# mbzuai-metaverse/XMem2

Hardware: AMD Instinct MI355X
Metric: frames/sec at 480p, 1 obj, 32 memory frames; mask IoU vs reference (higher is better)
Workload: dtype f32

## Files before the change

xmem2_amd/csrc/gemm_stream.hip:

```cpp
#include "gemm_stream.hpp"
#include <stdlib.h>

#ifdef XMEM_TOOLS
#define DBG(bit) (p.dbg & (bit))
#else
#define DBG(bit) 0
#endif

namespace {

__device__ __forceinline__ void glds16(const void* sbase, unsigned voff, unsigned lds_addr) {
    asm volatile("s_mov_b32 m0, %0\n\ts_nop 0\n\tglobal_load_lds_dwordx4 %1, %2" : : "s"(lds_addr), "v"(voff), "s"(sbase) : "memory");
}

template <int N>
__device__ __forceinline__ void wait_loads_only() {
    asm volatile("s_waitcnt vmcnt(%0)" : : "n"(N) : "memory");
}

template <int N>
__device__ __forceinline__ void wait_loads_then_barrier() {
    asm volatile("s_waitcnt vmcnt(%0)\n\ts_barrier" : : "n"(N) : "memory");
}

template <int TM, int TN, int NS, int MODE>
__global__ __launch_bounds__(256) void gemm_stream_kernel(GemmStreamArgs p) {
    constexpr int BM = 64 * TM, BN = 64 * TN;
    constexpr int STAGE = (BM + BN) * 128;
    constexpr int LA = BM / 32, LB = BN / 32;
    constexpr int L = LA + LB;
    extern __shared__ __attribute__((aligned(16))) unsigned char smem[];

    const int tid = threadIdx.x, lane = tid & 63;
    const int wave = __builtin_amdgcn_readfirstlane(tid >> 6);
    const int wm = wave >> 1, wn = wave & 1;
    const int l31 = lane & 31, lh = lane >> 5;

    int bid = blockIdx.x;
    {
        const int nwg = gridDim.x, q = nwg >> 3, r = nwg & 7, xcd = bid & 7;
        bid = (xcd < r ? xcd * (q + 1) : r * (q + 1) + (xcd - r) * q) + (bid >> 3);
    }
    const int ustep = DBG(32) ? 1 : (int)gridDim.x;
    const int u0 = DBG(32) ? bid * p.units_per_wg : bid;
    const int u1 = DBG(32) ? min(p.units, u0 + p.units_per_wg) : p.units;
    if (u0 >= u1) return;
    const int nunits = (u1 - u0 + ustep - 1) / ustep;
    const int S = nunits * p.nk;
    const unsigned lds_base = (unsigned)(size_t)smem;

    const int lrow = lane >> 3, lslot = lane & 7;
    unsigned a_voff[LA], b_voff[LB];
    int ld_u = u0, ld_kt = 0;
    const char* ld_abase = nullptr;
    const char* ld_bbase = nullptr;
    auto ld_unit_setup = [&]() {
        const int lu = DBG(1) ? 0 : ld_u;
        const int tn = lu % p.tiles_n, t2 = lu / p.tiles_n;
        const int tm = t2 % p.tiles_m, g = t2 / p.tiles_m;
        const int m0 = tm * BM, n0 = tn * BN;
#pragma unroll
        for (int i = 0; i < LA; ++i) {
            const int r = 8 * (4 * i + wave) + lrow;
            const int m = min(m0 + r, p.M - 1);
            unsigned row = (unsigned)m;
            if (MODE == 1 && p.stride != 1) {
                const int b = m / p.HoWo, rem = m - b * p.HoWo;
                const int oh = rem / p.Wo, ow = rem - oh * p.Wo;
                row = (unsigned)((b * p.H + oh * p.stride) * p.W + ow * p.stride);
            }
            a_voff[i] = (row * (unsigned)p.lda + (unsigned)((lslot ^ ((r >> 1) & 7)) * 4)) * 4u;
        }
#pragma unroll
        for (int i = 0; i < LB; ++i) {
            const int r = 8 * (4 * i + wave) + lrow;
            const int n = min(n0 + r, p.N - 1);
            b_voff[i] = ((unsigned)n * (unsigned)p.ldb + (unsigned)((lslot ^ ((r >> 1) & 7)) * 4)) * 4u;
        }
        ld_abase = reinterpret_cast<const char*>(p.A + (size_t)g * p.a_gstride);
        ld_bbase = reinterpret_cast<const char*>(p.B + (size_t)g * p.b_gstride);
    };
    auto issue = [&](int stage) {
        const char* ab = ld_abase + (size_t)ld_kt * 128;
        const char* bb = ld_bbase + (size_t)ld_kt * 128;
        const unsigned dst = lds_base + (unsigned)stage * STAGE + (unsigned)wave * 1024u;
#pragma unroll
        for (int i = 0; i < LA; ++i) glds16(ab, a_voff[i], dst + i * 4096);
#pragma unroll
        for (int i = 0; i < LB; ++i) glds16(bb, b_voff[i], dst + BM * 128 + i * 4096);
        if (++ld_kt == p.nk) {
            ld_kt = 0;
            ld_u += ustep;
            if (ld_u < u1) ld_unit_setup();
        }
    };

    const int swz = (l31 >> 1) & 7;
    unsigned rd_a[4], rd_b[4];
#pragma unroll
    for (int kk = 0; kk < 4; ++kk) {
        const unsigned ch = (unsigned)(((2 * kk + lh) ^ swz) * 16);
        rd_a[kk] = (unsigned)((wm * 32 * TM + l31) * 128) + ch;
        rd_b[kk] = (unsigned)(BM * 128 + (wn * 32 * TN + l31) * 128) + ch;
    }

    ld_unit_setup();
#pragma unroll
    for (int j = 0; j < NS - 1; ++j)
        if (j < S) issue(j);

    constexpr int ST = (MODE == 0) ? 16 * TM * TN : 0;
    constexpr int WAIT_STEADY = L * (NS - 2);
    constexpr int WAIT_CREDIT = (WAIT_STEADY + ST > 63) ? 63 : WAIT_STEADY + ST;
    int s = 0, stage = 0, credit = 0;
    for (int cu = u0; cu < u1; cu += ustep) {
        f32x16 acc[TM][TN];
#pragma unroll
        for (int i = 0; i < TM; ++i)
#pragma unroll
            for (int j = 0; j < TN; ++j)
#pragma unroll
                for (int r = 0; r < 16; ++r) acc[i][j][r] = 0.f;

        for (int kt = 0; kt < p.nk; ++kt, ++s) {
            const int behind = S - 1 - s;
            if (DBG(4)) wait_loads_only<WAIT_STEADY>();
            else if (behind >= NS - 2) {
                if (ST > 0 && credit > 0) wait_loads_then_barrier<WAIT_CREDIT>();
                else wait_loads_then_barrier<WAIT_STEADY>();
            } else if (NS > 3 && behind == 1) wait_loads_then_barrier<L>();
            else wait_loads_then_barrier<0>();
            if (credit > 0) --credit;
            if (s + NS - 1 < S && !DBG(8)) {
                int st = stage + NS - 1; if (st >= NS) st -= NS;
                issue(st);
            }

            const unsigned char* sb = smem + (DBG(16) ? 0 : stage * STAGE);
            f32x4 af[2][TM], bf[2][TN];
            if (DBG(16)) {
                const f32x4 c = {1.f, 2.f, 3.f, 4.f};
#pragma unroll
                for (int i = 0; i < TM; ++i) { af[0][i] = c; af[1][i] = c; }
#pragma unroll
                for (int j = 0; j < TN; ++j) { bf[0][j] = c; bf[1][j] = c; }
#pragma unroll
                for (int kk = 0; kk < 4; ++kk)
#pragma unroll
                    for (int t = 0; t < 4; ++t)
#pragma unroll
                        for (int i = 0; i < TM; ++i)
#pragma unroll
                            for (int j = 0; j < TN; ++j)
                                acc[i][j] = __builtin_amdgcn_mfma_f32_32x32x2f32(af[0][i][t], bf[0][j][t], acc[i][j], 0, 0, 0);
                if (++stage == NS) stage = 0;
                continue;
            }
#pragma unroll
            for (int i = 0; i < TM; ++i) af[0][i] = *reinterpret_cast<const f32x4*>(sb + rd_a[0] + i * 4096);
#pragma unroll
            for (int j = 0; j < TN; ++j) bf[0][j] = *reinterpret_cast<const f32x4*>(sb + rd_b[0] + j * 4096);
#pragma unroll
            for (int kk = 0; kk < 4; ++kk) {
                const int cur = kk & 1, nxt = cur ^ 1;
                if (kk + 1 < 4) {
#pragma unroll
                    for (int i = 0; i < TM; ++i) af[nxt][i] = *reinterpret_cast<const f32x4*>(sb + rd_a[kk + 1] + i * 4096);
#pragma unroll
                    for (int j = 0; j < TN; ++j) bf[nxt][j] = *reinterpret_cast<const f32x4*>(sb + rd_b[kk + 1] + j * 4096);
                }
                __builtin_amdgcn_sched_barrier(0);
                if (MODE == 1) {
#pragma unroll
                    for (int i = 0; i < TM; ++i) {
                        af[cur][i].x = fmaxf(af[cur][i].x, p.relu_in ? 0.f : af[cur][i].x); af[cur][i].y = fmaxf(af[cur][i].y, p.relu_in ? 0.f : af[cur][i].y);
                        af[cur][i].z = fmaxf(af[cur][i].z, p.relu_in ? 0.f : af[cur][i].z); af[cur][i].w = fmaxf(af[cur][i].w, p.relu_in ? 0.f : af[cur][i].w);
                    }
                }
#pragma unroll
                for (int t = 0; t < 4; ++t)
#pragma unroll
                    for (int i = 0; i < TM; ++i)
#pragma unroll
                        for (int j = 0; j < TN; ++j)
                            acc[i][j] = __builtin_amdgcn_mfma_f32_32x32x2f32(af[cur][i][t], bf[cur][j][t], acc[i][j], 0, 0, 0);
            }
            if (++stage == NS) stage = 0;
        }

        const int tn = cu % p.tiles_n, t2 = cu / p.tiles_n;
        const int tm = t2 % p.tiles_m, g = t2 / p.tiles_m;
        const int m0 = tm * BM, n0 = tn * BN;
        float* const cg = p.C + (size_t)g * p.c_gstride;
        bool all_full = true;
        if (DBG(2)) { credit = 0; continue; }
#pragma unroll
        for (int j = 0; j < TN; ++j) {
            const int nb = n0 + wn * 32 * TN + j * 32;
            const int n = nb + l31;
            float sc = 1.f, sh = 0.f;
            if (MODE == 1 && n < p.N) { sc = p.scale[n]; sh = p.shift[n]; }
#pragma unroll
            for (int i = 0; i < TM; ++i) {
                const int mw = m0 + wm * 32 * TM + i * 32;
                const int mb = mw + 4 * lh;
                float* const orow = cg + (size_t)mb * p.ldc + n;
                const bool full = (mw + 32 <= p.M) && (nb + 32 <= p.N);
                all_full = all_full && full;
                if (MODE == 0) {
                    if (full) {
#pragma unroll
                        for (int r = 0; r < 16; ++r) orow[(size_t)((r & 3) + 8 * (r >> 2)) * p.ldc] = acc[i][j][r];
                    } else if (n < p.N) {
#pragma unroll
                        for (int r = 0; r < 16; ++r) {
                            const int o = (r & 3) + 8 * (r >> 2);
                            if (mb + o < p.M) orow[(size_t)o * p.ldc] = acc[i][j][r];
                        }
                    }
                } else if (n < p.N) {
                    float rv[16];
                    if (p.res) {
#pragma unroll
                        for (int r = 0; r < 16; ++r) {
                            const int o = (r & 3) + 8 * (r >> 2);
                            const int t = p.res_mod ? (mb + o) % p.res_mod : min(mb + o, p.M - 1);
                            rv[r] = p.res[(size_t)t * p.ldres + n];
                        }
                    }
                    float vout[16];
#pragma unroll
                    for (int r = 0; r < 16; ++r) {
                        float v = acc[i][j][r] * sc + sh;
                        if (p.res) v += rv[r];
                        vout[r] = p.relu_out ? fmaxf(v, 0.f) : v;
                    }
#pragma unroll
                    for (int r = 0; r < 16; ++r) {
                        const int o = (r & 3) + 8 * (r >> 2);
                        if (mb + o < p.M) orow[(size_t)o * p.ldc] = vout[r];
                    }
                }
            }
        }
        credit = (ST > 0 && all_full) ? NS - 1 : 0;
    }
}

template <int TM, int TN, int NS>
int launch_variant(const GemmStreamArgs& a, int nwg, hipStream_t s) {
    const size_t lds = (size_t)NS * (64 * TM + 64 * TN) * 128;
    auto kern = a.mode == 1 ? gemm_stream_kernel<TM, TN, NS, 1> : gemm_stream_kernel<TM, TN, NS, 0>;
    if (xmem_ensure_dynamic_lds(reinterpret_cast<const void*>(kern), lds) != XMEM_OK) return XMEM_ERR_LAUNCH;
    hipLaunchKernelGGL(kern, dim3(nwg), dim3(256), lds, s, a);
    return xmem_check_launch();
}

}

size_t gemm_stream_lds_bytes(int variant, int ring) {
    const int bm = variant == 0 ? 64 : 128, bn = variant == 2 ? 128 : 64;
    return (size_t)ring * (bm + bn) * 128;
}

int gemm_stream_launch(GemmStreamArgs& a, int variant, int ring, hipStream_t s) {
    if (a.K % 32 != 0 || a.K <= 0 || a.M <= 0 || a.N <= 0 || a.G <= 0) return XMEM_ERR_UNSUPPORTED;
    if (variant < 0 || variant > 2 || (ring != 3 && ring != 4)) return XMEM_ERR_BAD_ARG;
    const int bm = variant == 0 ? 64 : 128, bn = variant == 2 ? 128 : 64;
    a.dbg = 0;
#ifdef XMEM_TOOLS
    { static const int dbg = getenv("XMEM_STREAM_DBG") ? atoi(getenv("XMEM_STREAM_DBG")) : 0; a.dbg = dbg; }
#endif
    a.nk = a.K / 32;
    a.tiles_m = cdiv(a.M, bm); a.tiles_n = cdiv(a.N, bn);
    const long units = (long)a.G * a.tiles_m * a.tiles_n;
    if (units > 0x7fffffff) return XMEM_ERR_UNSUPPORTED;
    a.units = (int)units;
    const size_t lds = gemm_stream_lds_bytes(variant, ring);
    int per_cu = (int)((160 * 1024) / lds); if (per_cu > 8) per_cu = 8; if (per_cu < 1) per_cu = 1;
    const int slots = 256 * per_cu;
    a.units_per_wg = cdiv(a.units, slots);
    const int nwg = cdiv(a.units, a.units_per_wg);
    if (variant == 0) return ring == 3 ? launch_variant<1, 1, 3>(a, nwg, s) : launch_variant<1, 1, 4>(a, nwg, s);
    if (variant == 1) return ring == 3 ? launch_variant<2, 1, 3>(a, nwg, s) : launch_variant<2, 1, 4>(a, nwg, s);
    return ring == 3 ? launch_variant<2, 2, 3>(a, nwg, s) : launch_variant<2, 2, 4>(a, nwg, s);
}
```

Baseline: 679.4.

## Use 8-wave workgroups for larger GEMM stream tiles

The streaming GEMM kernel is now templated on wave count. The larger tile variants (128x64, 128x128) use 512-thread workgroups with a 4x2 wave grid, each wave computing a 32-row slice, so per-wave accumulator count and register pressure drop. The 64x64 variant keeps 4 waves. Workgroup sizing for 8-wave variants now caps the grid at the slot count rather than rebalancing units per WG, and an environment override for the slot count is added. The trade is more waves sharing each LDS stage, which raises barrier cost per step.

```diff
diff --git a/xmem2_amd/csrc/gemm_stream.hip b/xmem2_amd/csrc/gemm_stream.hip
--- a/xmem2_amd/csrc/gemm_stream.hip
+++ b/xmem2_amd/csrc/gemm_stream.hip
@@ -23,11 +23,13 @@
     asm volatile("s_waitcnt vmcnt(%0)\n\ts_barrier" : : "n"(N) : "memory");
 }
 
-template <int TM, int TN, int NS, int MODE>
-__global__ __launch_bounds__(256) void gemm_stream_kernel(GemmStreamArgs p) {
-    constexpr int BM = 64 * TM, BN = 64 * TN;
+template <int NW, int TM, int TN, int NS, int MODE>
+__global__ __launch_bounds__(64 * NW) void gemm_stream_kernel(GemmStreamArgs p) {
+    static_assert(NW == 4 || NW == 8, "the wave grid is (NW / 2) x 2");
+    constexpr int BM = 32 * TM * (NW / 2), BN = 64 * TN;
     constexpr int STAGE = (BM + BN) * 128;
-    constexpr int LA = BM / 32, LB = BN / 32;
+    constexpr int LA = BM / (8 * NW), LB = BN / (8 * NW);
+    static_assert(LA * 8 * NW == BM && LB * 8 * NW == BN, "every wave issues the same number of LDS-DMA instructions per step");
     constexpr int L = LA + LB;
     extern __shared__ __attribute__((aligned(16))) unsigned char smem[];
 
@@ -61,7 +63,7 @@
         const int m0 = tm * BM, n0 = tn * BN;
 #pragma unroll
         for (int i = 0; i < LA; ++i) {
-            const int r = 8 * (4 * i + wave) + lrow;
+            const int r = 8 * (NW * i + wave) + lrow;
             const int m = min(m0 + r, p.M - 1);
             unsigned row = (unsigned)m;
             if (MODE == 1 && p.stride != 1) {
@@ -73,7 +75,7 @@
         }
 #pragma unroll
         for (int i = 0; i < LB; ++i) {
-            const int r = 8 * (4 * i + wave) + lrow;
+            const int r = 8 * (NW * i + wave) + lrow;
             const int n = min(n0 + r, p.N - 1);
             b_voff[i] = ((unsigned)n * (unsigned)p.ldb + (unsigned)((lslot ^ ((r >> 1) & 7)) * 4)) * 4u;
         }
@@ -85,9 +87,9 @@
         const char* bb = ld_bbase + (size_t)ld_kt * 128;
         const unsigned dst = lds_base + (unsigned)stage * STAGE + (unsigned)wave * 1024u;
 #pragma unroll
-        for (int i = 0; i < LA; ++i) glds16(ab, a_voff[i], dst + i * 4096);
-#pragma unroll
-        for (int i = 0; i < LB; ++i) glds16(bb, b_voff[i], dst + BM * 128 + i * 4096);
+        for (int i = 0; i < LA; ++i) glds16(ab, a_voff[i], dst + i * (NW * 1024));
+#pragma unroll
+        for (int i = 0; i < LB; ++i) glds16(bb, b_voff[i], dst + BM * 128 + i * (NW * 1024));
         if (++ld_kt == p.nk) {
             ld_kt = 0;
             ld_u += ustep;
@@ -247,14 +249,16 @@
     }
 }
 
-template <int TM, int TN, int NS>
+template <int NW, int TM, int TN, int NS>
 int launch_variant(const GemmStreamArgs& a, int nwg, hipStream_t s) {
-    const size_t lds = (size_t)NS * (64 * TM + 64 * TN) * 128;
-    auto kern = a.mode == 1 ? gemm_stream_kernel<TM, TN, NS, 1> : gemm_stream_kernel<TM, TN, NS, 0>;
+    const size_t lds = (size_t)NS * (32 * TM * (NW / 2) + 64 * TN) * 128;
+    auto kern = a.mode == 1 ? gemm_stream_kernel<NW, TM, TN, NS, 1> : gemm_stream_kernel<NW, TM, TN, NS, 0>;
     if (xmem_ensure_dynamic_lds(reinterpret_cast<const void*>(kern), lds) != XMEM_OK) return XMEM_ERR_LAUNCH;
-    hipLaunchKernelGGL(kern, dim3(nwg), dim3(256), lds, s, a);
+    hipLaunchKernelGGL(kern, dim3(nwg), dim3(64 * NW), lds, s, a);
     return xmem_check_launch();
 }
+
+constexpr int kCUs = 256;
 
 }
 
@@ -276,12 +280,23 @@
     const long units = (long)a.G * a.tiles_m * a.tiles_n;
     if (units > 0x7fffffff) return XMEM_ERR_UNSUPPORTED;
     a.units = (int)units;
+    const int nw = variant == 0 ? 4 : 8;
     const size_t lds = gemm_stream_lds_bytes(variant, ring);
-    int per_cu = (int)((160 * 1024) / lds); if (per_cu > 8) per_cu = 8; if (per_cu < 1) per_cu = 1;
-    const int slots = 256 * per_cu;
-    a.units_per_wg = cdiv(a.units, slots);
-    const int nwg = cdiv(a.units, a.units_per_wg);
-    if (variant == 0) return ring == 3 ? launch_variant<1, 1, 3>(a, nwg, s) : launch_variant<1, 1, 4>(a, nwg, s);
-    if (variant == 1) return ring == 3 ? launch_variant<2, 1, 3>(a, nwg, s) : launch_variant<2, 1, 4>(a, nwg, s);
-    return ring == 3 ? launch_variant<2, 2, 3>(a, nwg, s) : launch_variant<2, 2, 4>(a, nwg, s);
-}
+    int per_cu = (int)((160 * 1024) / lds); if (per_cu > 32 / nw) per_cu = 32 / nw; if (per_cu < 1) per_cu = 1;
+    int slots = kCUs * per_cu;
+    if (const char* e = getenv("XMEM_STREAM_SLOTS")) {
+        const int v = atoi(e);
+        if (v > 0 && v < slots) slots = v;
+    }
+    int nwg;
+    if (nw == 4) {
+        a.units_per_wg = cdiv(a.units, slots);
+        nwg = cdiv(a.units, a.units_per_wg);
+    } else {
+        nwg = a.units < slots ? a.units : slots;
+        a.units_per_wg = cdiv(a.units, nwg);
+    }
+    if (variant == 0) return ring == 3 ? launch_variant<4, 1, 1, 3>(a, nwg, s) : launch_variant<4, 1, 1, 4>(a, nwg, s);
+    if (variant == 1) return ring == 3 ? launch_variant<8, 1, 1, 3>(a, nwg, s) : launch_variant<8, 1, 1, 4>(a, nwg, s);
+    return ring == 3 ? launch_variant<8, 1, 2, 3>(a, nwg, s) : launch_variant<8, 1, 2, 4>(a, nwg, s);
+}
```

New measurement: 679.8, median of 3. No clear change (+0.1%).
